# tiantianz/redpanda

Hardware: AMD Instinct MI355X
Metric: validated+decoded batch GB/s per GPU and whole node; % of HBM peak (higher is better)
Workload: dtype u8

## Files before the change

### redpanda_amd/csrc/rp_internal.h

```cpp
#pragma once

#include <hip/hip_runtime.h>
#include <stdint.h>

#include "rpgpu.h"

namespace rp {

constexpr uint64_t kNone = ~0ull;
constexpr uint32_t kCrcPoly = 0x82F63B78u;

constexpr uint32_t kShiftLevels = 6;
constexpr uint32_t kBraidSkip = 1020;

constexpr uint32_t kVWaves = 16;
constexpr uint32_t kWinBytes = 16384;
constexpr uint32_t kLdsBraidOff = 0;
constexpr uint32_t kLdsSlice4Off = 131072;
constexpr uint32_t kLdsShiftOff = kLdsSlice4Off + 4096;
constexpr uint32_t kLdsValidateBytes = kLdsShiftOff + kShiftLevels * 4096;
static_assert(kLdsValidateBytes <= 160u * 1024u, "validate LDS image exceeds 160 KiB");

struct Tables {
    uint32_t slice[4][256];
// ... 87 lines not shown
    uint64_t tab;
    uint64_t s0[4];
    uint32_t sn[4];
    uint32_t cnt[4];
    uint32_t lsz, seg, ns, hlog, x2;
    uint32_t status;
};
constexpr uint32_t kZsPlanned = 5;
constexpr uint32_t kZsExact = 6, kZsExactAgain = 7;

struct GzsItem {
    uint32_t member;
    uint32_t k, nk;
    int32_t status;
    uint64_t begin, end;
    uint64_t start;
    uint64_t stop;
    uint64_t out;
    uint64_t len;
    uint64_t guess;
    uint32_t cap, pad;
};
#ifndef RPGPU_GZS_MIN
#define RPGPU_GZS_MIN 16384
#endif
#ifndef RPGPU_GZS_CHUNK
#define RPGPU_GZS_CHUNK 16384
#endif
constexpr uint64_t kGzsMin = RPGPU_GZS_MIN;
constexpr uint64_t kGzsChunk = RPGPU_GZS_CHUNK;
constexpr uint32_t kGzsMaxK = 256;

constexpr size_t kCounterBytes = 256;

struct DeviceJob {
    const uint8_t* data;
    uint64_t data_len;
    const uint64_t* seg_off;
    const uint64_t* chunk_base;
    uint32_t n_segments;
    uint32_t flags;
    uint32_t layout;
    uint32_t chunk_bytes;
    uint32_t total_chunks;
    ChunkRec* chunks;
    uint64_t* chunk_count;
    uint64_t* chunk_entry;
    SegTerm* seg_term;
    rpgpu_batch_result* batches;
    uint64_t batch_capacity;
    uint64_t* slots;
    uint64_t* dcap;
    rpgpu_record_index* records;
    uint64_t record_capacity;
    uint8_t* decoded;
    uint64_t decoded_capacity;
    rpgpu_segment_summary* summaries;
    rpgpu_job_totals* totals;
    uint64_t* bitmap;
    const Tables* tables;
    uint32_t* counters;
    uint32_t* decode_list;
    uint32_t* seq_list;
    uint32_t* link_list;
    uint32_t* long_list;
    uint32_t* wlong_list;
// ... 8 lines not shown
    uint32_t crc_compose;
    uint32_t* dchain;
    uint32_t* slab_next;
    uint32_t pool_slabs;
    uint2* frecs;
    uint64_t frec_cap;
    uint32_t* lzf_list;
    uint32_t* lane_list;
    uint32_t* raw_list;
    uint32_t* lzf_tail;
    BlockItem* blocks;
    uint32_t block_capacity;
    FramePlan* plans;
    uint32_t* seg_first_bad;
    const uint64_t* seeds;
    const uint64_t* seed_off;
    uint32_t* inf_list;
    uint32_t* inf_state;
    uint64_t* inf_off;
    uint64_t* inf_total;
    uint8_t* inf_scratch;
    uint64_t inf_scratch_bytes;
    uint64_t* inf_scratch_used;
    uint32_t zs_fast;
    uint32_t zs_split;
    uint64_t* zs_items;
    uint32_t zs_items_cap;
    uint32_t* host_list;
    uint32_t* gzs_mem;
    GzsItem* gzs_items;
    uint32_t gzs_items_cap;
    uint16_t* gzs_pool;
    uint64_t gzs_pool_syms;
};

struct HostItem {
    uint64_t src;
    uint64_t stage;
    uint64_t out_len;
    uint64_t cap;
    uint32_t n;
    uint32_t ord;
    int32_t record_count;
    int32_t status;
};
hipError_t launch_host_desc(const DeviceJob& j, HostItem* items, uint32_t n, hipStream_t s);
hipError_t launch_host_gather(const DeviceJob& j, const HostItem* items, uint32_t n, uint8_t* stage, hipStream_t s);
hipError_t launch_host_patch(const DeviceJob& j, const HostItem* items, uint32_t n, hipStream_t s);
hipError_t launch_host_scatter(const DeviceJob& j, const HostItem* items, uint32_t n, const uint8_t* stage,
                               hipStream_t s);

hipError_t launch_chunk_base(const DeviceJob& j, hipStream_t s);
hipError_t launch_discover(const DeviceJob& j, hipStream_t s);
hipError_t launch_resolve(const DeviceJob& j, hipStream_t s);
hipError_t launch_emit(const DeviceJob& j, hipStream_t s);
hipError_t launch_validate(const DeviceJob& j, hipStream_t s, uint32_t grid, bool compose = true);
hipError_t launch_crc_compose(const DeviceJob& j, hipStream_t s, uint32_t grid);
bool dchain_wanted(const DeviceJob& j);
hipError_t launch_dchain(const DeviceJob& j, hipStream_t s, uint32_t grid);
hipError_t launch_validate_decoded(const DeviceJob& j, hipStream_t s, uint32_t grid);
hipError_t launch_walk(const DeviceJob& j, hipStream_t s, uint32_t grid);
hipError_t launch_decode(const DeviceJob& j, hipStream_t s, uint32_t grid);
hipError_t launch_decode_blocks(const DeviceJob& j, hipStream_t s, uint32_t grid);
hipError_t launch_lz_walk(const DeviceJob& j, hipStream_t s, uint32_t grid);
hipError_t launch_lz_exec(const DeviceJob& j, hipStream_t s);
hipError_t launch_raw_copy(const DeviceJob& j, hipStream_t s, uint32_t cus);
// ... 83 lines not shown
```

### redpanda_amd/csrc/rp_kernels.hip

```cpp
#include "rp_device.h"

namespace rp {


#ifdef RPGPU_CHECKED
#include <cstdio>
#define RP_CHECK(flag, cond, fmt, ...)                                               \
    do {                                                                            \
        if (!(cond)) {                                                              \
            if (__lane_id() == 0) printf("RPGPU_CHECK %d " fmt "\n", __LINE__, __VA_ARGS__); \
            flag = true;                                                            \
        }                                                                           \
    } while (0)
#endif

DEV uint32_t find_segment(const uint64_t* __restrict__ chunk_base, uint32_t nseg, uint64_t g) {
    uint32_t lo = 0, hi = nseg;
    while (hi - lo > 1) {
        uint32_t mid = (lo + hi) >> 1;
        if (chunk_base[mid] <= g) lo = mid; else hi = mid;
    }
    return lo;
}

// ... 358 lines not shown
                }
                s_T = o.exit;
            }
        }
        __syncthreads();
        w0 = wf + 1;
    }
    for (uint64_t w = w0 + tid; w < W; w += 256) {
        if (s_ended) {
            j.chunk_count[c0 + w] = 0;
            j.chunk_entry[c0 + w] = kNone;
        }
    }
    if (tid == 0) {
        if (!s_ended) { s_st.pos = s_T; s_st.errc = RPGPU_ERRC_END_OF_STREAM; s_st.eof = 1; }
        j.seg_term[s] = s_st;
    }
}

__global__ __launch_bounds__(256) void k_emit(DeviceJob j) {
    extern __shared__ uint32_t th[];
    init_lds_hdr(th, j.tables);
    const uint64_t g = (uint64_t)blockIdx.x * blockDim.x + threadIdx.x;
    if (g >= j.total_chunks) return;
    const uint64_t base_ord = j.chunk_count[g];
    const uint64_t cnt = j.chunk_count[g + 1] - base_ord;
    if (cnt == 0) return;
    const uint32_t s = find_segment(j.chunk_base, j.n_segments, g);
    const uint64_t off = j.seg_off[s], len = j.seg_off[s + 1] - off;
    const uint8_t* seg = j.data + off;
    const uint32_t c57 = j.tables->c57;
    const bool wire = j.layout == RPGPU_LAYOUT_WIRE;
    uint64_t p = j.chunk_entry[g];
    for (uint64_t i = 0; i < cnt; i++) {
#ifdef RPGPU_CHECKED
        if (!(p < len)) {
            printf("RPGPU_CHECK emit g=%llu i=%llu cnt=%llu p=%llu len=%llu\n", (unsigned long long)g,
                   (unsigned long long)i, (unsigned long long)cnt, (unsigned long long)p, (unsigned long long)len);
            break;
        }
#endif
        const LHdr h = lane_header(j.layout, seg, len, p, th, c57);
        const uint64_t ord = base_ord + i;
        const bool complete = (len - p - RPGPU_HEADER_SIZE) >= h.need;
        const uint32_t praw = lane_prefix_raw(j.layout, h.w, th);
        const uint32_t attrs = wire ? lbe16(h.w, 21) : l16(h.w, 21);
        const int32_t rc = (int32_t)(wire ? lbe32(h.w, 57) : l32(h.w, 57));
        const uint32_t codec = attrs & 7;
        uint64_t slots = 0, cap = 0;
        const bool decodable = (codec == RPGPU_CODEC_LZ4 || codec == RPGPU_CODEC_SNAPPY) && (j.flags & RPGPU_JOB_DECODE);
        if (complete) {
            if (codec == 0) {
                if ((j.flags & RPGPU_JOB_PARSE) && rc > 0 && (uint64_t)rc <= h.need) slots = (uint64_t)rc;
            } else if (decodable) {
                cap = decode_capacity_dev((int)codec, seg + p + RPGPU_HEADER_SIZE, h.need);
                if ((j.flags & RPGPU_JOB_PARSE) && rc > 0 && (uint64_t)rc <= cap) slots = (uint64_t)rc;
            }
        }
        if (ord < j.batch_capacity) {
            rpgpu_batch_result r;
            r.file_pos = p;
            uint32_t f = RPGPU_F_HEADER_OK;
            if (wire) {
                r.base_offset = (int64_t)lbe64(h.w, 0);
                r.first_timestamp = (int64_t)lbe64(h.w, 27);
                r.max_timestamp = (int64_t)lbe64(h.w, 35);
// ... 11 lines not shown
                r.max_timestamp = (int64_t)l64(h.w, 35);
                r.producer_id = (int64_t)l64(h.w, 43);
                r.last_offset_delta = (int32_t)l32(h.w, 23);
                r.base_sequence = (int32_t)l32(h.w, 53);
                r.header_crc = h.hcrc;
                r.crc = l32(h.w, 17);
                r.producer_epoch = (int16_t)l16(h.w, 51);
                r.type = (int8_t)lb(h.w, 16);
            }
            r.size_bytes = h.size;
            r.record_count = rc;
            r.crc_computed = 0;
            r.header_crc_computed = h.computed;
            if (complete) f |= RPGPU_F_COMPLETE;
            if (codec) f |= RPGPU_F_COMPRESSED;
            if (codec >= 5) f |= RPGPU_F_CODEC_INVALID;
            const bool host_codec = (j.flags & RPGPU_JOB_DECODE) && (j.flags & RPGPU_JOB_HOST_CODECS);
            if (complete && codec == RPGPU_CODEC_ZSTD && !(j.flags & RPGPU_JOB_DECODE)) f |= RPGPU_F_CODEC_UNSUPPORTED;
            r.flags = f;
            r.segment = s;
            r.index_base = off + p + RPGPU_HEADER_SIZE;
            r.decoded_off = 0;
            r.records_parsed = 0;
            r.decoded_len = (complete && codec == 0) ? (uint32_t)h.need : 0;
            r.decoded_crc = 0;
            r.decoded_header_crc = 0;
            r.attrs = (int16_t)attrs;
            r.parse_err = 0;
            r.reserved0 = 0;
            r.reserved1 = praw;
            j.batches[ord] = r;
            j.slots[ord] = slots;
            j.dcap[ord] = cap;
            if (complete && decodable) j.decode_list[atomicAdd(&j.counters[2], 1u)] = (uint32_t)ord;
            if (complete && (j.flags & RPGPU_JOB_DECODE) &&
                (codec == RPGPU_CODEC_GZIP || (codec == RPGPU_CODEC_ZSTD && !host_codec)))
                j.inf_list[atomicAdd(&j.counters[16], 1u)] = (uint32_t)ord;
            if (complete && codec == RPGPU_CODEC_ZSTD && host_codec)
                j.host_list[atomicAdd(&j.counters[19], 1u)] = (uint32_t)ord;
        }
        if (!complete) break;
        p += RPGPU_HEADER_SIZE + h.need;
    }
}

constexpr uint32_t kScanTile = 4096;

__global__ __launch_bounds__(256) void k_scan_tiles(uint64_t* data, const uint64_t* d_n, uint64_t n_host, uint64_t* tile_sums) {
    const uint64_t n = d_n ? (*d_n < n_host ? *d_n : n_host) : n_host;
    const uint64_t t0 = (uint64_t)blockIdx.x * kScanTile;
    if (t0 >= n) return;
    __shared__ uint64_t s[256];
    uint64_t v[16];
    uint64_t sum = 0;
    const uint64_t b = t0 + threadIdx.x * 16;
#pragma unroll
    for (int i = 0; i < 16; i++) {
        v[i] = (b + i < n) ? data[b + i] : 0;
        sum += v[i];
    }
    s[threadIdx.x] = sum;
    __syncthreads();
    for (int o = 1; o < 256; o <<= 1) {
        uint64_t x = (threadIdx.x >= (uint32_t)o) ? s[threadIdx.x - o] : 0;
        __syncthreads();
        s[threadIdx.x] += x;
        __syncthreads();
    }
    uint64_t run = s[threadIdx.x] - sum;
#pragma unroll
    for (int i = 0; i < 16; i++) {
        if (b + i < n) data[b + i] = run;
        run += v[i];
    }
    if (threadIdx.x == 255) tile_sums[blockIdx.x] = s[255];
}
// ... 83 lines not shown
        sm.has_checkpoint = 0;
        sm.ckpt_last_offset = 0;
        sm.ckpt_truncate_pos = 0;
        if (fits && bad > 0) {
            const rpgpu_batch_result& g = j.batches[first + bad - 1];
            sm.has_checkpoint = 1;
            sm.ckpt_last_offset = (int64_t)((uint64_t)g.base_offset + (uint64_t)(int64_t)g.last_offset_delta);
            sm.ckpt_truncate_pos = s_phys;
        }
        const uint64_t sf = first < j.batch_capacity ? first : j.batch_capacity;
        const uint64_t sl = last < j.batch_capacity ? last : j.batch_capacity;
        sm.n_records = j.slots[sl] - j.slots[sf];
        sm.reserved[0] = sm.reserved[1] = 0;
        j.summaries[s] = sm;
    }
}

DEV bool batch_valid(uint32_t f, uint32_t job_flags, uint32_t layout) {
    if (layout == RPGPU_LAYOUT_WIRE && !(f & RPGPU_F_WIRE_V2)) return false;
    if (!(f & RPGPU_F_HEADER_OK) || !(f & RPGPU_F_COMPLETE) || !(f & RPGPU_F_CRC_OK)) return false;
    if (f & RPGPU_F_CODEC_INVALID) return false;
    if ((f & RPGPU_F_COMPRESSED) && (job_flags & RPGPU_JOB_DECODE) && !(f & RPGPU_F_CODEC_UNSUPPORTED) &&
        !(f & RPGPU_F_CODEC_OK))
        return false;
    if ((f & RPGPU_F_PARSED) && !(f & RPGPU_F_PARSE_OK)) return false;
    return true;
}

__global__ __launch_bounds__(256) void k_finalize_bitmap(DeviceJob j) {
    const uint64_t nb_total = j.chunk_count[j.total_chunks];
    const uint64_t nb = nb_total < j.batch_capacity ? nb_total : j.batch_capacity;
    const uint64_t b = (uint64_t)blockIdx.x * 256 + threadIdx.x;
    if ((b & ~63ull) >= nb) return;
    const uint64_t word = __ballot(b < nb && batch_valid(j.batches[b].flags, j.flags, j.layout));
    if ((threadIdx.x & 63) == 0) j.bitmap[b >> 6] = word;
}

__global__ void k_finalize_totals(DeviceJob j) {
    if (threadIdx.x != 0 || blockIdx.x != 0) return;
    const uint64_t nb_total = j.chunk_count[j.total_chunks];
    const uint64_t nb = nb_total < j.batch_capacity ? nb_total : j.batch_capacity;
    rpgpu_job_totals t;
    t.n_batches = nb_total;
    t.n_records = j.slots[nb];
    const uint64_t dtot = (j.flags & RPGPU_JOB_DECODE) ? j.dcap[nb] : 0;
    t.decoded_bytes = dtot;
    t.batch_capacity_needed = nb_total;
    t.record_capacity_needed = j.slots[nb];
    t.decoded_capacity_needed = dtot;
    uint32_t ov = j.counters[1];
    if (nb_total > j.batch_capacity) ov |= 1;
    if (j.slots[nb] > j.record_capacity) ov |= 2;
    if (dtot > j.decoded_capacity) ov |= 4;
    t.overflow = ov;
    t.n_rewalks = j.counters[0];
    t.reserved[0] = t.reserved[1] = 0;
    *j.totals = t;
}

__global__ __launch_bounds__(256) void k_host_desc(DeviceJob j, HostItem* items) {
    const uint32_t i = blockIdx.x * blockDim.x + threadIdx.x;
    if (i >= j.counters[19]) return;
    const uint32_t b = j.host_list[i];
    const rpgpu_batch_result& R = j.batches[b];
    HostItem it;
    it.src = j.seg_off[R.segment] + R.file_pos + RPGPU_HEADER_SIZE;
    it.n = (uint32_t)(R.size_bytes - (int32_t)RPGPU_HEADER_SIZE);
    it.ord = b;
// ... 83 lines not shown
            __syncthreads();
        }
        if (i < j.n_segments) ((uint64_t*)j.chunk_base)[i] = carry + sh[threadIdx.x] - v;
        __syncthreads();
        if (threadIdx.x == 1023) carry += sh[1023];
        __syncthreads();
    }
    if (threadIdx.x == 0) ((uint64_t*)j.chunk_base)[j.n_segments] = carry;
}

hipError_t launch_chunk_base(const DeviceJob& j, hipStream_t s) {
    hipLaunchKernelGGL(k_chunk_base, dim3(1), dim3(1024), 0, s, j);
    return hipGetLastError();
}

hipError_t launch_discover(const DeviceJob& j, hipStream_t s) {
    hipLaunchKernelGGL(k_discover, dim3((j.total_chunks + 3) / 4), dim3(256), 0, s, j);
    hipError_t e = hipGetLastError();
    if (e != hipSuccess) return e;
    hipLaunchKernelGGL(k_chain, dim3((j.total_chunks + 255) / 256), dim3(256), kLdsHdrBytes, s, j);
    return hipGetLastError();
}
hipError_t launch_resolve(const DeviceJob& j, hipStream_t s) {
    hipLaunchKernelGGL(k_resolve, dim3(j.n_segments), dim3(256), 0, s, j);
    return hipGetLastError();
}
hipError_t launch_emit(const DeviceJob& j, hipStream_t s) {
    hipLaunchKernelGGL(k_emit, dim3((j.total_chunks + 255) / 256), dim3(256), kLdsHdrBytes, s, j);
    return hipGetLastError();
}
hipError_t launch_finalize(const DeviceJob& j, hipStream_t s) {
    hipLaunchKernelGGL(k_finalize_segments, dim3(j.n_segments), dim3(256), 0, s, j);
    const uint64_t words = (j.batch_capacity + 63) / 64;
    if (j.bitmap) {
        const uint32_t grid = (uint32_t)((words * 64 + 255) / 256);
        hipLaunchKernelGGL(k_finalize_bitmap, dim3(grid ? grid : 1), dim3(256), 0, s, j);
    }
    hipLaunchKernelGGL(k_finalize_totals, dim3(1), dim3(64), 0, s, j);
    return hipGetLastError();
}

size_t scan_temp_bytes(uint64_t n) { return ((n + kScanTile - 1) / kScanTile + 1) * sizeof(uint64_t); }

hipError_t scan_exclusive_dev(uint64_t* data, const uint64_t* d_n, uint64_t n_cap, uint64_t* temp, hipStream_t s) {
    const uint32_t tiles = (uint32_t)((n_cap + kScanTile - 1) / kScanTile);
    const uint32_t g = tiles ? tiles : 1;
    hipLaunchKernelGGL(k_scan_tiles, dim3(g), dim3(256), 0, s, data, d_n, n_cap, temp);
    hipLaunchKernelGGL(k_scan_sums, dim3(1), dim3(1024), 0, s, temp, d_n, n_cap, temp + g);
    hipLaunchKernelGGL(k_scan_add, dim3(g), dim3(256), 0, s, data, d_n, n_cap, temp);
    return hipGetLastError();
}

__global__ void k_copy_total(uint64_t* data, const uint64_t* d_n, uint64_t n_host, const uint64_t* total) {
    const uint64_t n = d_n ? (*d_n < n_host ? *d_n : n_host) : n_host;
    data[n] = *total;
}

hipError_t scan_exclusive_u64(uint64_t* data, uint64_t n, void* temp, size_t temp_bytes, hipStream_t s) {
    (void)temp_bytes;
    uint64_t* t = (uint64_t*)temp;
    const uint32_t tiles = (uint32_t)((n + kScanTile - 1) / kScanTile);
    scan_exclusive_dev(data, nullptr, n, t, s);
    hipLaunchKernelGGL(k_copy_total, dim3(1), dim3(1), 0, s, data, (const uint64_t*)nullptr, n, t + (tiles ? tiles : 1));
    return hipGetLastError();
}

hipError_t scan_exclusive_u64_devn(uint64_t* data, const uint64_t* d_n, uint64_t n_cap, void* temp, hipStream_t s) {
// ... 9 lines not shown
```

### redpanda_amd/csrc/rp_runtime.hip

```cpp
#include <hip/hip_runtime.h>
#include <nmmintrin.h>

#include <algorithm>
#include <array>
#include <atomic>
#include <cstdio>
#include <cstdlib>
#include <cstring>
#include <mutex>
#include <random>
#include <string>
#include <thread>
#include <vector>

#include "rp_device.h"
#include "rp_hostcodec.h"

namespace rp {

static uint32_t raw_step_zero(uint32_t c, const uint32_t* t0) { return t0[c & 0xFF] ^ (c >> 8); }

static void build_tables(Tables* T) {
    uint32_t t0[256];
    for (uint32_t i = 0; i < 256; i++) {
// ... 561 lines not shown
        it.cap = it.status == 0 ? align_up(it.out_len, 16) : 0;
        it.stage = out_total;
        out_total += it.cap;
    }
    if (int rc = grow_staging(c, c->hc_out, out_total + 16, s)) return rc;
    if (int rc = grow_staging(c, c->hc_out_h, out_total + 16, s)) return rc;
    for (uint32_t i = 0; i < n; i++)
        if (hit[i].status == 0) memcpy((uint8_t*)c->hc_out_h.p + hit[i].stage, outs[i].data(), hit[i].out_len);
    HIPCHK(c, hipMemcpyAsync(c->hc_out.p, c->hc_out_h.p, out_total, hipMemcpyHostToDevice, s));
    HIPCHK(c, hipMemcpyAsync(dit, hit, ib, hipMemcpyHostToDevice, s));
    HIPCHK(c, launch_host_patch(j, dit, n, s));
    c->hc_n = n;
    return RPGPU_OK;
}

int check_job(rpgpu_ctx* c, const rpgpu_job* job) {
    if (!c || !job || !job->d_data || !job->d_seg_offsets || !job->h_seg_offsets || job->n_segments == 0 ||
        !job->d_batches || !job->d_summaries || !job->d_totals)
        return fail(c, RPGPU_E_INVALID, "rpgpu_submit: missing argument");
    if (((uintptr_t)job->d_data & 15) != 0) return fail(c, RPGPU_E_INVALID, "rpgpu_submit: d_data must be 16-byte aligned");
    if (job->layout != RPGPU_LAYOUT_DISK && job->layout != RPGPU_LAYOUT_WIRE)
        return fail(c, RPGPU_E_INVALID, "rpgpu_submit: unknown layout");
    if ((job->flags & RPGPU_JOB_PARSE) && !job->d_records && job->record_capacity)
        return fail(c, RPGPU_E_INVALID, "rpgpu_submit: PARSE needs d_records");
    return RPGPU_OK;
}

struct Layout {
    uint64_t tc;
    uint64_t zcap, gcap, bl_cap, split_min, split_cap;
    size_t cbase, chunks, ccount, centry, segterm, slots, dcap, counters, dlist, slist, llist, fbad;
    size_t ilist, istate, ioff, itot, hlist, zitems, gzsmem, gzsit;
    size_t blocks, plans, pstate, longl, wlong, rawl, lanel, lzfl, lzft, split, spart, scan;
    size_t need;
};

Layout job_layout(const rpgpu_job* job, uint32_t cu_count) {
    Layout L;
    const uint32_t nseg = job->n_segments;
    const uint32_t cs = job->chunk_bytes ? job->chunk_bytes : (256u << 10);
    const uint64_t bcap = job->batch_capacity, data_len = job->h_seg_offsets[nseg];
    uint64_t tc = 0;
    for (uint32_t i = 0; i < nseg; i++) {
        const uint64_t len = job->h_seg_offsets[i + 1] - job->h_seg_offsets[i];
        uint64_t nc = (len + cs - 1) / cs;
        tc += nc ? nc : 1;
    }
    L.tc = tc;
    size_t off = 0;
    auto take = [&](size_t bytes) { size_t o = off; off = align_up(off + bytes, 256); return o; };
    L.cbase = take((nseg + 1) * 8);
    L.chunks = take(tc * sizeof(ChunkRec));
    L.ccount = take((tc + 1) * 8);
    L.centry = take(tc * 8);
    L.segterm = take(nseg * sizeof(SegTerm));
    L.slots = take((bcap + 1) * 8);
    L.dcap = take((bcap + 1) * 8);
    L.counters = take(kCounterBytes);
    L.dlist = take((bcap + 1) * 4);
    L.slist = take((bcap + 1) * 4);
    L.llist = take((bcap + 1) * 4);
    L.fbad = take((size_t)nseg * 4);
    const bool decode_job = (job->flags & RPGPU_JOB_DECODE) != 0;
    L.ilist = take(decode_job ? (bcap + 1) * 4 : 0);
    L.istate = take(decode_job ? (bcap + 1) * 4 : 0);
    L.ioff = take(decode_job ? (bcap + 1) * 8 : 0);
    L.itot = take(decode_job ? (bcap + 1) * 8 : 0);
    const bool host_job = decode_job && (job->flags & RPGPU_JOB_HOST_CODECS);
    L.hlist = take(host_job ? (bcap + 1) * 4 : 0);
    L.zcap = decode_job ? std::min<uint64_t>(data_len / 16384 + 8 * bcap + 64, 0x7FFFFFFFull) : 0;
    L.zitems = take(L.zcap * 8);
    L.gzsmem = take(decode_job ? 2 * (bcap + 1) * 4 : 0);
    L.gcap = decode_job ? std::min<uint64_t>(data_len / kGzsChunk + bcap + 64, 0x7FFFFFFFull) : 0;
    L.gzsit = take(L.gcap * sizeof(GzsItem));
    const bool dec = decode_job && job->d_decoded;
    L.bl_cap = dec ? std::min<uint64_t>(data_len / 16384 + 2 * bcap + 64, 0x7FFFFFFFull) : 0;
    L.blocks = take(L.bl_cap * sizeof(BlockItem));
    L.plans = take(dec ? (bcap + 1) * sizeof(FramePlan) : 0);
    L.pstate = take(L.bl_cap * sizeof(PieceState));
    L.longl = take(L.bl_cap * 4);
    L.wlong = take(L.bl_cap * 4);
    L.rawl = take(L.bl_cap * 4);
    L.lanel = take(L.bl_cap * 4);
    L.lzfl = take(L.bl_cap * 4);
    L.lzft = take(L.bl_cap * 4);
    L.split_min = diag().split_min ? diag().split_min
                                   : std::max<uint64_t>(kSplitMin, 2 * data_len / ((uint64_t)cu_count * kVWaves));
    L.split_cap = std::min<uint64_t>(data_len / L.split_min + 1, bcap + 1);
    L.split = take(L.split_cap * 4);
    L.spart = take(L.split_cap * kSplitParts * 4);
    L.scan = take(scan_temp_bytes(std::max<uint64_t>(tc, bcap)) + 64);
    L.need = off;
    return L;
}

int bind_job(rpgpu_ctx* c, const rpgpu_job* job, const Layout& L, hipStream_t s, int stop, DeviceJob& j) {
    const uint32_t nseg = job->n_segments;
    const uint64_t data_len = job->h_seg_offsets[nseg];
    const bool dec = (job->flags & RPGPU_JOB_DECODE) && job->d_decoded;
    if (dec && !c->seqs.p) {
        const uint32_t waves = c->cu_count * lz_exec_wgs_per_cu();
        if (int rc = grow(c, c->seqs, (size_t)waves * kRecsPerLane * sizeof(SeqRec), s, "decode sequence workspace")) return rc;
        c->exec_waves = waves;
    }
    const size_t slab_bytes = kSlabRecs * sizeof(SeqRec) + 4;
    const size_t pool_want = dec ? std::min<size_t>(std::max<size_t>(data_len / 2, 256ull << 20), 8ull << 30) : 0;
    if (int rc = grow(c, c->pool, pool_want, s, "decode record pool")) return rc;
    if (int rc = grow(c, c->ws, L.need, s, "workspace")) return rc;
    uint8_t* ws = c->ws.as<uint8_t>();

    j.data = job->d_data;
    j.data_len = data_len;
    j.seg_off = job->d_seg_offsets;
    j.chunk_base = (const uint64_t*)(ws + L.cbase);
    j.n_segments = nseg;
    j.flags = job->flags;
    j.layout = job->layout;
    j.chunk_bytes = job->chunk_bytes ? job->chunk_bytes : (256u << 10);
    j.total_chunks = (uint32_t)L.tc;
    j.chunks = (ChunkRec*)(ws + L.chunks);
    j.chunk_count = (uint64_t*)(ws + L.ccount);
    j.chunk_entry = (uint64_t*)(ws + L.centry);
    j.seg_term = (SegTerm*)(ws + L.segterm);
    j.batches = job->d_batches;
// ... 55 lines not shown
    j.inf_scratch_used = (uint64_t*)(j.counters + 24);
    if (dec && stop == kRunAll) {
        const size_t want = diag().inf_pool ? diag().inf_pool
                                            : std::min<size_t>(std::max<size_t>(2 * data_len, 256ull << 20), 2ull << 30);
        if (int rc = grow_optional(c, c->gz_pool, want, s)) return rc;
        if (c->gz_pool.p) {
            j.inf_scratch = c->gz_pool.as<uint8_t>();
            j.inf_scratch_bytes = std::min<size_t>(c->gz_pool.bytes, want);
        }
    }
    j.zs_fast = diag().zs_fast;
    j.zs_split = 0;
    j.zs_items = (uint64_t*)(ws + L.zitems);
    j.zs_items_cap = (uint32_t)L.zcap;
    j.host_list = (uint32_t*)(ws + L.hlist);
    j.gzs_mem = nullptr;
    j.gzs_items = (GzsItem*)(ws + L.gzsit);
    j.gzs_items_cap = (uint32_t)L.gcap;
    j.gzs_pool = nullptr;
    j.gzs_pool_syms = 0;
    if (j.inf_scratch && diag().gzs && L.gcap) {
        const size_t want = std::min<size_t>(std::max<size_t>(2 * data_len, 64ull << 20), 4ull << 30);
        if (int rc = grow_optional(c, c->gzs_pool, want, s)) return rc;
        if (c->gzs_pool.p) {
            j.gzs_mem = (uint32_t*)(ws + L.gzsmem);
            j.gzs_pool = c->gzs_pool.as<uint16_t>();
            j.gzs_pool_syms = c->gzs_pool.bytes / 2;
        }
    }
    c->hc_n = 0;
    j.blocks = (BlockItem*)(ws + L.blocks);
    j.block_capacity = (uint32_t)L.bl_cap;
    j.plans = (FramePlan*)(ws + L.plans);
    if (((uintptr_t)job->d_decoded & 15) != 0) return fail(c, RPGPU_E_INVALID, "rpgpu_submit: d_decoded must be 16-byte aligned");
    return RPGPU_OK;
}

#define STAGE(name, call)                                                                  \
    do {                                                                                   \
        HIPCHK(c, (call));                                                                 \
        if (diag().debug_sync) {                                                           \
            fprintf(stderr, "[rpgpu] stage %s\n", name);                                   \
            fflush(stderr);                                                                \
            hipError_t _e = hipStreamSynchronize(s);                                       \
            if (_e == hipSuccess && c->side.stream) _e = hipStreamSynchronize(c->side.stream);   \
            if (_e == hipSuccess && c->side2.stream) _e = hipStreamSynchronize(c->side2.stream); \
            if (_e != hipSuccess) return fail(c, RPGPU_E_HIP, "stage " name " failed", _e); \
        }                                                                                  \
    } while (0)

hipError_t mark(hipEvent_t* ev, int i, hipStream_t s) { return ev ? hipEventRecord(ev[i], s) : hipSuccess; }

int stage_discover(rpgpu_ctx* c, const DeviceJob& j, hipStream_t s, hipEvent_t* ev, uint64_t* scan_tmp, bool emit) {
    STAGE("chunk_base", launch_chunk_base(j, s));
    HIPCHK(c, hipMemsetAsync(j.counters, 0, kCounterBytes, s));
    HIPCHK(c, hipMemsetAsync(j.seg_first_bad, 0xFF, (size_t)j.n_segments * 4, s));
    STAGE("discover", launch_discover(j, s));
    HIPCHK(c, mark(ev, 1, s));
    STAGE("resolve", launch_resolve(j, s));
    STAGE("scan_chunks", scan_exclusive_u64(j.chunk_count, j.total_chunks, scan_tmp, 0, s));
    if (emit) STAGE("emit", launch_emit(j, s));
    return RPGPU_OK;
}

int stage_members(rpgpu_ctx* c, DeviceJob& j, hipStream_t s, uint64_t* scan_tmp) {
    const uint32_t cus = c->cu_count;
// ... 844 lines not shown
```

### redpanda_amd/csrc/rp_validate.hip

```cpp
#include "rp_device.h"

namespace rp {

#ifdef RPGPU_STAMPS
__device__ unsigned long long g_stamps[8];
__shared__ unsigned long long s_stamps[kVWaves][8];
#define STAMP(v) const uint64_t v = __builtin_amdgcn_s_memtime()
#define STAMP_ADD(i, d) do { if (lane() == 0) s_stamps[threadIdx.x >> 6][i] += (unsigned long long)(d); } while (0)
#else
#define STAMP(v)
#define STAMP_ADD(i, d)
#endif

DEV uint32_t L32(const uint8_t* lds, uint32_t a) { return *(const uint32_t*)(lds + a); }

DEV uint32_t lane_v() {
    uint32_t r;
    asm volatile("v_mbcnt_lo_u32_b32 %0, -1, 0\n\tv_mbcnt_hi_u32_b32 %0, -1, %0" : "=v"(r));
    return r;
}

typedef const __attribute__((address_space(4))) uint32_t cu32;

struct Keys {
// ... 503 lines not shown
}

DEV uint32_t decoded_header_crc(const Tables* T, const uint8_t* hdr, uint32_t new_size, uint32_t new_crc,
                                bool wire) {
    const uint32_t l = lane_v();
    uint32_t b = (l < RPGPU_HEADER_SIZE) ? (uint32_t)hdr[l] : 0u;
    if (wire) {
        int src = 0;
        if (l >= 8 && l < 16) src = 15 - (int)l;
        else if (l >= 17 && l < 21) src = 37 - (int)l;
        else if (l >= 21 && l < RPGPU_HEADER_SIZE) src = 21 + be_index(l);
        b = (uint32_t)__shfl((int)b, src, 64);
        if (l == 16) b = 1u;
    }
    if (l >= 4 && l < 8) b = (new_size >> (8 * (l - 4))) & 0xFFu;
    if (l >= 17 && l < 21) b = (new_crc >> (8 * (l - 17))) & 0xFFu;
    if (l == 21) b &= ~7u;
    uint32_t x = (l >= 4 && l < RPGPU_HEADER_SIZE) ? T->hdr[60 - l][b] : 0u;
    x ^= swz_xor<1>(x);
    x ^= swz_xor<2>(x);
    x ^= swz_xor<4>(x);
    x ^= swz_xor<8>(x);
    x ^= swz_xor<16>(x);
    return ~(T->c57 ^ rl(x, 0) ^ rl(x, 32));
}

DEV void note_bad(const DeviceJob& j, uint32_t seg, uint64_t b) {
    if (lane_v() == 0) {
        const uint64_t first = j.chunk_count[j.chunk_base[seg]];
        atomicMin(&j.seg_first_bad[seg], (uint32_t)(b - first));
    }
}

#ifndef RPGPU_LANE_WALK_MAX
#define RPGPU_LANE_WALK_MAX 256
#endif
constexpr int32_t kLaneWalkMax = RPGPU_LANE_WALK_MAX;
DEV bool lane_walked(uint32_t flags, uint32_t codec, int32_t rc) {
    return (flags & RPGPU_F_COMPLETE) && codec == 0 && rc <= kLaneWalkMax;
}

constexpr int kDwSize = offsetof(rpgpu_batch_result, size_bytes) / 4;
constexpr int kDwCount = offsetof(rpgpu_batch_result, record_count) / 4;
constexpr int kDwCrc = offsetof(rpgpu_batch_result, crc) / 4;
constexpr int kDwFlags = offsetof(rpgpu_batch_result, flags) / 4;
constexpr int kDwSeg = offsetof(rpgpu_batch_result, segment) / 4;
constexpr int kDwBase = offsetof(rpgpu_batch_result, index_base) / 4;
constexpr int kDwDlen = offsetof(rpgpu_batch_result, decoded_len) / 4;
constexpr int kDwAttrs = offsetof(rpgpu_batch_result, attrs) / 4;
constexpr int kDwPraw = offsetof(rpgpu_batch_result, reserved1) / 4;
constexpr int kDwRes0 = offsetof(rpgpu_batch_result, reserved0) / 4;
constexpr int kDwCcomp = offsetof(rpgpu_batch_result, crc_computed) / 4;
static_assert(offsetof(rpgpu_batch_result, reserved0) % 4 == 2, "reserved0: the high half of its dword");
static_assert(sizeof(rpgpu_batch_result) == 128 && offsetof(rpgpu_batch_result, attrs) % 4 == 0, "desc layout");

DEV uint32_t load_desc_raw(const DeviceJob& j, uint64_t b) {
    const uint32_t l = lane_v();
    const uint32_t* p = l < 32u ? (const uint32_t*)&j.batches[b] + l
                      : l < 34u ? (const uint32_t*)&j.slots[b] + (l - 32u)
                      : l < 36u ? (const uint32_t*)&j.slots[b + 1] + (l - 34u)
                                : (const uint32_t*)&j.dcap[b] + (l & 1u);
    return l < 38u ? *p : 0u;
}

struct Desc {
    uint32_t flags, crc, praw, codec, seg, dlen;
    uint64_t S, n, ib, islots, doff;
    int32_t rc;
    uint32_t scc;
    uint32_t ccomp;
};

DEV Desc desc_of(uint32_t raw) {
// ... 290 lines not shown
        e.hdr_count = r.hcount;
        e.hdr_pos = r.hdr_pos;
        e.end_pos = r.end;
        e.attrs = (int8_t)r.attr;
        e.pad[0] = e.pad[1] = e.pad[2] = 0;
        e.reserved[0] = e.reserved[1] = 0;
        dst = w.out + w.done;
    }
    w.done++;
    w.start = r.end;
    if (w.done >= w.total) {
        wr.parsed = w.done;
        wr.err = 0;
        wr.trailing = n - w.start;
        return true;
    }
    const uint32_t g = w.start + mis;
    fresh = g - cb > kRegionReach;
    w.h_base = fresh ? (g & ~15u) : cb;
    return false;
}

struct WalkCtx {
    const uint8_t* data;
    const uint64_t* seg_off;
    rpgpu_batch_result* batches;
    const uint64_t* slots;
    rpgpu_record_index* records;
    uint64_t record_capacity;
    uint32_t* counters;
    const uint64_t* chunk_count;
    const uint64_t* chunk_base;
    uint32_t* seg_first_bad;
};

DEV WalkCtx walk_ctx(const DeviceJob& j) {
    return WalkCtx{j.data, j.seg_off, j.batches, j.slots, j.records, j.record_capacity, j.counters,
                   j.chunk_count, j.chunk_base, j.seg_first_bad};
}

DEV bool lane_walk_setup(const WalkCtx& j, uint64_t b, LaneWalk& w, bool& idx_ok) {
    const rpgpu_batch_result* R = &j.batches[b];
    const int32_t rc = R->record_count;
    if (!lane_walked(R->flags, (uint32_t)R->attrs & 7u, rc)) return false;
    const uint64_t S = j.seg_off[R->segment] + R->file_pos + RPGPU_HEADER_SIZE;
    const uint32_t n = (uint32_t)(R->size_bytes - (int32_t)RPGPU_HEADER_SIZE);
    const uint64_t ib = j.slots[b], islots = j.slots[b + 1] - ib;
    idx_ok = ib + islots <= j.record_capacity;
    lane_walk_begin(w, j.data + S, n, rc, (uint32_t)b, idx_ok ? j.records + ib : nullptr,
                    idx_ok ? (uint32_t)islots : 0u);
    return true;
}

DEV void lane_walk_finish(const WalkCtx& j, uint64_t b, const WalkResult& w, bool idx_ok, bool wire) {
    rpgpu_batch_result* R = &j.batches[b];
    uint32_t f = RPGPU_F_PARSED, perr = w.err;
    if (perr == 0) {
        f |= RPGPU_F_PARSE_ASYNC_OK;
        if (w.trailing == 0) f |= RPGPU_F_PARSE_OK;
        else perr = RPGPU_PARSE_ERR_TRAILING;
    }
    if (f & RPGPU_F_PARSE_OK) {
        if (idx_ok) f |= RPGPU_F_INDEX_WRITTEN;
        else { perr = RPGPU_PARSE_ERR_INDEX_CAPACITY; atomicOr(&j.counters[1], 2u); }
    }
    if (wire && !(f & RPGPU_F_PARSE_OK)) note_bad_lane(j, R->segment, b);
    atomicOr(&R->flags, f);
    R->records_parsed = w.parsed;
    R->parse_err = (uint8_t)perr;
}

__global__ __launch_bounds__(1024) void k_validate(DeviceJob j) {
    extern __shared__ __attribute__((aligned(16))) uint8_t lds[];
    const Tables* T = j.tables;
    const uint32_t tid = threadIdx.x;
    init_lds_tables(lds, T);
    const uint32_t l = lane_v();
    const Keys K = make_keys();
    const uint32_t c40 = uni32(T->c40);

    const uint64_t nb_total = j.chunk_count[j.total_chunks];
    const uint64_t nb = nb_total < j.batch_capacity ? nb_total : j.batch_capacity;
    const uint64_t nw = (uint64_t)gridDim.x * kVWaves;
#ifdef RPGPU_STAMPS
    if (l == 0)
        for (int i = 0; i < 8; i++) s_stamps[tid >> 6][i] = 0;
#endif
    STAMP(tk0);
    uint64_t b = (uint64_t)blockIdx.x * kVWaves + (tid >> 6);
    if (b < nb) {
        uint32_t raw = load_desc_raw(j, b);
        Desc dn = desc_of(raw);
        Stream sn = stored_stream(j, dn, true);
        Win v;
        load_rows<0, kPreRows>(sn, v);
        for (; b < nb; b += nw) {
            const Desc d = dn;
            const Stream st = sn;
            const uint64_t bn = b + nw;
            const bool more = bn < nb;
            raw = load_desc_raw(j, more ? bn : b);
            load_rows<kPreRows, 16>(st, v);
// ... 289 lines not shown
            R->reserved0 = 0;
            R->reserved1 = 0;
        }
    }
}

__global__ __launch_bounds__(256) void k_walk(DeviceJob j) {
    extern __shared__ __attribute__((aligned(16))) uint8_t lds[];
    enum : uint32_t { kIdle = 0, kHead = 1, kWalk = 2, kFin = 3 };
    uint8_t* wave = lds + (threadIdx.x >> 6) * kWalkLdsWave;
    const uint32_t l = lane_v();
    const uint64_t nb_total = j.chunk_count[j.total_chunks];
    const uint64_t nb = nb_total < j.batch_capacity ? nb_total : j.batch_capacity;
    const bool wire = j.layout == RPGPU_LAYOUT_WIRE;
    const uint64_t stride = (uint64_t)gridDim.x * blockDim.x;
    const WalkCtx c = walk_ctx(j);
    uint64_t b = (uint64_t)blockIdx.x * blockDim.x + threadIdx.x;
    uint32_t st = kIdle;
    bool first = true, idx_ok = false;
    LaneWalk w;
    for (uint32_t step = 0;; step++) {
        uint8_t* hslot = wave + (step & 1u) * kSlotBytes;
        uint8_t* cslot = wave + (~step & 1u) * kSlotBytes;
        if (st == kIdle) {
            if (!first) b += stride;
            first = false;
            if (b >= nb) st = kFin;
            else if (!(wire && !(j.batches[b].flags & RPGPU_F_CRC_OK)) && lane_walk_setup(c, b, w, idx_ok)) {
                if (w.total == 0) {
                    WalkResult wr;
                    wr.parsed = 0; wr.err = 0; wr.trailing = w.n;
                    lane_walk_finish(c, b, wr, idx_ok, wire);
                } else st = kHead;
            }
        }
        uint32_t want = 0, rows = 0;
        if (st == kWalk) want = lane_c_base(w, hslot + region_lane(l));
        else if (st == kHead) want = w.h_base;
        if (st == kWalk || st == kHead) rows = region_rows(w.n, w.mis, want);
        if (__ballot(st != kFin) == 0) break;
        if (kCoopLoad) coop_load(cslot, w.p0 - w.mis + want, rows);
        else {
            const uint8_t* g = w.p0 - w.mis + want;
#pragma unroll
            for (uint32_t r = 0; r < kRegionRows; r++)
                if (r < rows)
                    __builtin_amdgcn_global_load_lds((gbl_void*)(g + 16u * r), (lds_void*)(cslot + 1024u * r), 16, 0, 0);
        }
        wait_vm();
        rpgpu_record_index e;
        rpgpu_record_index* dst = nullptr;
        if (st == kWalk) {
            WalkResult wr;
            bool fresh = false;
            if (lane_record_step(w, wr, hslot + region_lane(l), cslot + region_lane(l), want, fresh, e, dst)) {
                lane_walk_finish(c, b, wr, idx_ok, wire);
                st = kIdle;
            } else if (fresh) st = kHead;
        } else if (st == kHead) st = kWalk;
        coop_store(hslot, e, dst);
    }
}

DEV uint32_t be40_src(uint32_t k) {
    return k < 2 ? 22 - k : k < 6 ? 26 - (k - 2) : k < 14 ? 34 - (k - 6) : k < 22 ? 42 - (k - 14) : k < 30 ? 50 - (k - 22)
         : k < 32 ? 52 - (k - 30) : k < 36 ? 56 - (k - 32) : 60 - (k - 36);
// ... 198 lines not shown
```

Measured before the change: 3436.

## Feed lane walker from compact per-batch descriptors and defer verdict merge to finalize

k_emit now writes a packed 16-byte WalkDesc per batch (start, size, record count or a not-walked mark), buffered four at a time. The lane walker reads that descriptor in place of scattered fields of the wide batch_result plus seg_off, which removes several dependent gathers per lane. Walk outcomes are written as one packed 64-bit verdict instead of an atomicOr and field stores on batch_result, and k_finalize_bitmap merges them later. This adds two workspace arrays, extra writes in emit, and a bitmap kernel launch for every parse job.

```diff
diff --git a/redpanda_amd/csrc/rp_internal.h b/redpanda_amd/csrc/rp_internal.h
--- a/redpanda_amd/csrc/rp_internal.h
+++ b/redpanda_amd/csrc/rp_internal.h
@@ -143,6 +143,29 @@
 constexpr uint32_t kGzsMaxK = 256;
 
 constexpr size_t kCounterBytes = 256;
+
+#ifndef RPGPU_LANE_WALK_MAX
+#define RPGPU_LANE_WALK_MAX 256
+#endif
+constexpr int32_t kLaneWalkMax = RPGPU_LANE_WALK_MAX;
+__host__ __device__ __forceinline__ bool lane_walked(uint32_t flags, uint32_t codec, int32_t rc) {
+    return (flags & RPGPU_F_COMPLETE) && codec == 0 && rc <= kLaneWalkMax;
+}
+
+struct WalkDesc {
+    uint64_t start;
+    uint32_t n;
+    int32_t rc;
+};
+static_assert(sizeof(WalkDesc) == 16, "one dwordx4 per lane");
+constexpr int32_t kNotLaneWalked = 0x7FFFFFFF;
+static_assert(kLaneWalkMax < kNotLaneWalked, "the mark is no record count k_walk takes");
+
+constexpr uint64_t kVerdictWalked = 1ull << 63;
+__host__ __device__ __forceinline__ uint64_t walk_verdict_pack(uint32_t flags, uint32_t parsed, uint32_t perr) {
+    return kVerdictWalked | ((uint64_t)(perr & 0x7Fu) << 56) | ((uint64_t)(parsed & 0xFFFFFFu) << 32) | flags;
+}
+static_assert(kLaneWalkMax <= 0xFFFFFF, "records_parsed field of the verdict");
 
 struct DeviceJob {
     const uint8_t* data;
@@ -217,6 +240,8 @@
     uint32_t gzs_items_cap;
     uint16_t* gzs_pool;
     uint64_t gzs_pool_syms;
+    WalkDesc* walk_desc;
+    uint64_t* walk_verdict;
 };
 
 struct HostItem {
diff --git a/redpanda_amd/csrc/rp_kernels.hip b/redpanda_amd/csrc/rp_kernels.hip
--- a/redpanda_amd/csrc/rp_kernels.hip
+++ b/redpanda_amd/csrc/rp_kernels.hip
@@ -414,6 +414,15 @@
     const uint32_t c57 = j.tables->c57;
     const bool wire = j.layout == RPGPU_LAYOUT_WIRE;
     uint64_t p = j.chunk_entry[g];
+    WalkDesc wq[4];
+    uint32_t wn = 0;
+    uint64_t wfirst = 0;
+    auto wflush = [&]() __attribute__((always_inline)) {
+#pragma unroll
+        for (uint32_t k = 0; k < 4; k++)
+            if (k < wn) j.walk_desc[wfirst + k] = wq[k];
+        wn = 0;
+    };
     for (uint64_t i = 0; i < cnt; i++) {
 #ifdef RPGPU_CHECKED
         if (!(p < len)) {
@@ -491,6 +500,18 @@
             j.batches[ord] = r;
             j.slots[ord] = slots;
             j.dcap[ord] = cap;
+            if (j.flags & RPGPU_JOB_PARSE) {
+                WalkDesc wd;
+                wd.start = r.index_base;
+                wd.n = (uint32_t)(h.size - (int32_t)RPGPU_HEADER_SIZE);
+                wd.rc = lane_walked(f, codec, rc) ? rc : kNotLaneWalked;
+                if (wn == 0) wfirst = ord;
+#pragma unroll
+                for (uint32_t k = 0; k < 4; k++)
+                    if (k == wn) wq[k] = wd;
+                wn++;
+                if ((ord & 3u) == 3u) wflush();
+            }
             if (complete && decodable) j.decode_list[atomicAdd(&j.counters[2], 1u)] = (uint32_t)ord;
             if (complete && (j.flags & RPGPU_JOB_DECODE) &&
                 (codec == RPGPU_CODEC_GZIP || (codec == RPGPU_CODEC_ZSTD && !host_codec)))
@@ -501,6 +522,7 @@
         if (!complete) break;
         p += RPGPU_HEADER_SIZE + h.need;
     }
+    wflush();
 }
 
 constexpr uint32_t kScanTile = 4096;
@@ -650,8 +672,20 @@
     const uint64_t nb = nb_total < j.batch_capacity ? nb_total : j.batch_capacity;
     const uint64_t b = (uint64_t)blockIdx.x * 256 + threadIdx.x;
     if ((b & ~63ull) >= nb) return;
-    const uint64_t word = __ballot(b < nb && batch_valid(j.batches[b].flags, j.flags, j.layout));
-    if ((threadIdx.x & 63) == 0) j.bitmap[b >> 6] = word;
+    uint32_t f = 0;
+    if (b < nb) {
+        rpgpu_batch_result* R = &j.batches[b];
+        f = R->flags;
+        const uint64_t v = (j.flags & RPGPU_JOB_PARSE) ? j.walk_verdict[b] : 0;
+        if (v & kVerdictWalked) {
+            f |= (uint32_t)v;
+            R->flags = f;
+            R->records_parsed = (uint32_t)(v >> 32) & 0xFFFFFFu;
+            R->parse_err = (uint8_t)((v >> 56) & 0x7Fu);
+        }
+    }
+    const uint64_t word = __ballot(b < nb && batch_valid(f, j.flags, j.layout));
+    if (j.bitmap && (threadIdx.x & 63) == 0) j.bitmap[b >> 6] = word;
 }
 
 __global__ void k_finalize_totals(DeviceJob j) {
@@ -801,7 +835,7 @@
 hipError_t launch_finalize(const DeviceJob& j, hipStream_t s) {
     hipLaunchKernelGGL(k_finalize_segments, dim3(j.n_segments), dim3(256), 0, s, j);
     const uint64_t words = (j.batch_capacity + 63) / 64;
-    if (j.bitmap) {
+    if (j.bitmap || (j.flags & RPGPU_JOB_PARSE)) {
         const uint32_t grid = (uint32_t)((words * 64 + 255) / 256);
         hipLaunchKernelGGL(k_finalize_bitmap, dim3(grid ? grid : 1), dim3(256), 0, s, j);
     }
diff --git a/redpanda_amd/csrc/rp_runtime.hip b/redpanda_amd/csrc/rp_runtime.hip
--- a/redpanda_amd/csrc/rp_runtime.hip
+++ b/redpanda_amd/csrc/rp_runtime.hip
@@ -617,6 +617,7 @@
     size_t cbase, chunks, ccount, centry, segterm, slots, dcap, counters, dlist, slist, llist, fbad;
     size_t ilist, istate, ioff, itot, hlist, zitems, gzsmem, gzsit;
     size_t blocks, plans, pstate, longl, wlong, rawl, lanel, lzfl, lzft, split, spart, scan;
+    size_t wdesc, wverd;
     size_t need;
 };
 
@@ -675,6 +676,9 @@
     L.split = take(L.split_cap * 4);
     L.spart = take(L.split_cap * kSplitParts * 4);
     L.scan = take(scan_temp_bytes(std::max<uint64_t>(tc, bcap)) + 64);
+    const bool parse_job = (job->flags & RPGPU_JOB_PARSE) != 0;
+    L.wdesc = take(parse_job ? (bcap + 1) * sizeof(WalkDesc) : 0);
+    L.wverd = take(parse_job ? (bcap + 1) * 8 : 0);
     L.need = off;
     return L;
 }
@@ -796,6 +800,8 @@
     j.blocks = (BlockItem*)(ws + L.blocks);
     j.block_capacity = (uint32_t)L.bl_cap;
     j.plans = (FramePlan*)(ws + L.plans);
+    j.walk_desc = (WalkDesc*)(ws + L.wdesc);
+    j.walk_verdict = (uint64_t*)(ws + L.wverd);
     if (((uintptr_t)job->d_decoded & 15) != 0) return fail(c, RPGPU_E_INVALID, "rpgpu_submit: d_decoded must be 16-byte aligned");
     return RPGPU_OK;
 }
diff --git a/redpanda_amd/csrc/rp_validate.hip b/redpanda_amd/csrc/rp_validate.hip
--- a/redpanda_amd/csrc/rp_validate.hip
+++ b/redpanda_amd/csrc/rp_validate.hip
@@ -559,13 +559,6 @@
     }
 }
 
-#ifndef RPGPU_LANE_WALK_MAX
-#define RPGPU_LANE_WALK_MAX 256
-#endif
-constexpr int32_t kLaneWalkMax = RPGPU_LANE_WALK_MAX;
-DEV bool lane_walked(uint32_t flags, uint32_t codec, int32_t rc) {
-    return (flags & RPGPU_F_COMPLETE) && codec == 0 && rc <= kLaneWalkMax;
-}
 
 constexpr int kDwSize = offsetof(rpgpu_batch_result, size_bytes) / 4;
 constexpr int kDwCount = offsetof(rpgpu_batch_result, record_count) / 4;
@@ -922,28 +915,26 @@
     const uint64_t* chunk_count;
     const uint64_t* chunk_base;
     uint32_t* seg_first_bad;
+    const WalkDesc* desc;
+    uint64_t* verdict;
 };
 
 DEV WalkCtx walk_ctx(const DeviceJob& j) {
     return WalkCtx{j.data, j.seg_off, j.batches, j.slots, j.records, j.record_capacity, j.counters,
-                   j.chunk_count, j.chunk_base, j.seg_first_bad};
+                   j.chunk_count, j.chunk_base, j.seg_first_bad, j.walk_desc, j.walk_verdict};
 }
 
 DEV bool lane_walk_setup(const WalkCtx& j, uint64_t b, LaneWalk& w, bool& idx_ok) {
-    const rpgpu_batch_result* R = &j.batches[b];
-    const int32_t rc = R->record_count;
-    if (!lane_walked(R->flags, (uint32_t)R->attrs & 7u, rc)) return false;
-    const uint64_t S = j.seg_off[R->segment] + R->file_pos + RPGPU_HEADER_SIZE;
-    const uint32_t n = (uint32_t)(R->size_bytes - (int32_t)RPGPU_HEADER_SIZE);
+    const WalkDesc d = j.desc[b];
+    if (d.rc == kNotLaneWalked) return false;
     const uint64_t ib = j.slots[b], islots = j.slots[b + 1] - ib;
     idx_ok = ib + islots <= j.record_capacity;
-    lane_walk_begin(w, j.data + S, n, rc, (uint32_t)b, idx_ok ? j.records + ib : nullptr,
+    lane_walk_begin(w, j.data + d.start, d.n, d.rc, (uint32_t)b, idx_ok ? j.records + ib : nullptr,
                     idx_ok ? (uint32_t)islots : 0u);
     return true;
 }
 
 DEV void lane_walk_finish(const WalkCtx& j, uint64_t b, const WalkResult& w, bool idx_ok, bool wire) {
-    rpgpu_batch_result* R = &j.batches[b];
     uint32_t f = RPGPU_F_PARSED, perr = w.err;
     if (perr == 0) {
         f |= RPGPU_F_PARSE_ASYNC_OK;
@@ -954,10 +945,8 @@
         if (idx_ok) f |= RPGPU_F_INDEX_WRITTEN;
         else { perr = RPGPU_PARSE_ERR_INDEX_CAPACITY; atomicOr(&j.counters[1], 2u); }
     }
-    if (wire && !(f & RPGPU_F_PARSE_OK)) note_bad_lane(j, R->segment, b);
-    atomicOr(&R->flags, f);
-    R->records_parsed = w.parsed;
-    R->parse_err = (uint8_t)perr;
+    if (wire && !(f & RPGPU_F_PARSE_OK)) note_bad_lane(j, j.batches[b].segment, b);
+    j.verdict[b] = walk_verdict_pack(f, w.parsed, perr);
 }
 
 __global__ __launch_bounds__(1024) void k_validate(DeviceJob j) {
@@ -1313,6 +1302,8 @@
                     wr.parsed = 0; wr.err = 0; wr.trailing = w.n;
                     lane_walk_finish(c, b, wr, idx_ok, wire);
                 } else st = kHead;
+            } else {
+                c.verdict[b] = 0;
             }
         }
         uint32_t want = 0, rows = 0;
```

Measured after the change: 3486 (median of 6 runs). 1.5% higher.
